# soasme/LTX-Video-GPUPoor

Measured on AMD Instinct MI355X. Metric: denoise-steps/sec + VAE-decode frames/sec, LTX-Video 768x512x97f at 1/8 GPU, higher is better.
Workload: dtype bf16

## Files before the change

### include/ltxmi.h

```cpp
#ifndef LTXMI_H
#define LTXMI_H

#include <stddef.h>
#include <stdint.h>

#ifdef __cplusplus
extern "C" {
#endif

typedef enum ltxmi_status {
    LTXMI_OK = 0,
    LTXMI_ERR_INVALID_ARG = -1,
    LTXMI_ERR_UNSUPPORTED = -2,
    LTXMI_ERR_LAUNCH = -3
} ltxmi_status;

const char* ltxmi_version(void);
const char* ltxmi_last_error(void);
const char* ltxmi_arch(void);

typedef enum ltxmi_epilogue {
    LTXMI_EPI_NONE = 0,
    LTXMI_EPI_GELU_TANH = 1,
    LTXMI_EPI_SILU = 2,
// ... 54 lines not shown
    const void* v; int64_t v_stride_b, v_stride_l;
    void*       o; int64_t o_stride_b, o_stride_l;
    const float* key_bias; int64_t bias_stride_b;
    int32_t B, H, Lq, Lk, head_dim;
    float   softmax_scale;
    const float* q_rowsumsq; int64_t q_rowsumsq_stride_b, q_rowsumsq_stride_l; int32_t q_rowsumsq_blocks;
    const void*  q_norm_weight; float q_norm_eps;
    const void*  rope_cos; const void* rope_sin; int64_t rope_stride_b, rope_stride_l;
    int32_t o_segment_len; int64_t o_stride_segment;
    const float* q_rstd; int64_t q_rstd_stride_b, q_rstd_stride_l;
    uint32_t* redo_counter; int32_t force_exact;
    float* lse; int64_t lse_stride_b, lse_stride_h;
} ltxmi_attn_args;

int ltxmi_attention_fwd_bf16(const ltxmi_attn_args* args, void* stream);
int ltxmi_attention_fuses_qnorm(int32_t B, int32_t H, int32_t Lq, int32_t Lk, int32_t head_dim, int32_t has_key_bias);
int ltxmi_attention_kernel_id(int32_t B, int32_t H, int32_t Lq, int32_t Lk, int32_t head_dim, int32_t has_key_bias,
                              int64_t k_stride_l, int64_t v_stride_l);

#define LTXMI_ATTN_MERGE_MAX 8
typedef struct ltxmi_attn_merge_args {
    int32_t n;
    const void*  o_part[LTXMI_ATTN_MERGE_MAX];   int64_t o_part_stride_b[LTXMI_ATTN_MERGE_MAX], o_part_stride_l[LTXMI_ATTN_MERGE_MAX];
    const float* lse_part[LTXMI_ATTN_MERGE_MAX]; int64_t lse_part_stride_b[LTXMI_ATTN_MERGE_MAX], lse_part_stride_h[LTXMI_ATTN_MERGE_MAX];
    void*  o;   int64_t o_stride_b, o_stride_l;
    float* lse; int64_t lse_stride_b, lse_stride_h;
    int32_t B, H, Lq, head_dim;
} ltxmi_attn_merge_args;
int ltxmi_attention_merge_bf16(const ltxmi_attn_merge_args* args, void* stream);

// ... 105 lines not shown
```

### ltx-video-gpupoor_amd/csrc/attention.h

```cpp
#pragma once
#include "common.h"

namespace ltxmi {

struct AttnParams {
    const uint16_t* q; int64_t q_sb, q_sl;
    const uint16_t* k; int64_t k_sb, k_sl;
    const uint16_t* v; int64_t v_sb, v_sl;
    uint16_t* o; int64_t o_sb, o_sl;
    const float* bias; int64_t bias_sb;
    int B, H, Lq, Lk;
    float scale_log2e;
    int q_tiles;
    const float* q_ss; int64_t q_ss_sb, q_ss_sl; int q_ss_n;
    const float* q_rstd; int64_t q_rstd_sb, q_rstd_sl;
    const uint16_t* q_w; float q_eps;
    const uint16_t* rope_cos; const uint16_t* rope_sin; int64_t rope_sb, rope_sl;
    int o_seg; int64_t o_sseg;
    uint32_t* redo_count; int force_exact;
    float* lse; int64_t lse_sb, lse_sh;

    __host__ __device__ __forceinline__ bool q_on_load() const { return q_ss != nullptr || q_rstd != nullptr; }
    __device__ __forceinline__ float q_row_rstd(int b, int row, int HD) const {
        if (q_rstd) return q_rstd[(int64_t)b * q_rstd_sb + (int64_t)row * q_rstd_sl];
// ... 146 lines not shown
}

template <typename Kern, typename... Extra>
static inline int attn_launch(Kern kern, int lds, unsigned long long* lds_done, AttnParams p, int tiles, hipStream_t stream,
                              Extra... extra) {
    if (const int rc = reserve_lds((const void*)kern, lds, lds_done, "ltxmi_attention_fwd_bf16")) return rc;
    p.q_tiles = tiles;
    const int64_t grid = (int64_t)p.B * p.H * tiles;
    hipLaunchKernelGGL(kern, dim3((unsigned)grid), dim3(256), lds, stream, p, extra...);
    return check_launch("ltxmi_attention_fwd_bf16");
}

int launch_attn_pipe(AttnParams p, hipStream_t stream);
int launch_attn_pipe128(AttnParams p, hipStream_t stream);
int launch_attn_cross(AttnParams p, hipStream_t stream);

}
```

### ltx-video-gpupoor_amd/csrc/attention.hip

```cpp
#include <type_traits>

#include "attention.h"

namespace ltxmi {

constexpr int KV_TILE = 64;
constexpr int Q_PER_WAVE = 32;
constexpr int Q_PER_WG = 128;
constexpr float LOG2E = 1.4426950408889634f;
constexpr int ATTN_QB_BIG = 2;

template <int DH>
struct AttnCfg {
    static constexpr int ROW_BYTES = DH * 2;
    static constexpr int TILE_BYTES = KV_TILE * DH * 2;
    static constexpr int CHUNKS_PER_ROW = DH / 8;
    static constexpr int LD_PER_THREAD = (KV_TILE * CHUNKS_PER_ROW) / 256;
    static constexpr int KSTEPS = DH / 16;
    static constexpr int DBLK = DH / 32;
    static constexpr int BIAS_BYTES = KV_TILE * 4;
    static constexpr int STAGE_BYTES = 2 * TILE_BYTES + BIAS_BYTES;
    static constexpr int SMEM = 2 * STAGE_BYTES;
    __device__ static __forceinline__ int k_swz(int row) {
        return DH == 64 ? ((row >> 1) & 7) : (row & 15);
// ... 329 lines not shown
    const bool span_ok = (rows * k_sl + head_dim) * 2 < (1ll << 31) && (rows * v_sl + head_dim) * 2 < (1ll << 31);
    if (head_dim == 128) {
        if (!has_bias && wg256 >= 128 && Lk >= 1024 && span_ok) return ATTN_PIPE128;
        return has_bias ? ATTN_DH128_BIAS : ATTN_DH128;
    }
    if (Lk <= ATTN_CROSS_MAX_KEYS && Lq >= 1024) return ATTN_CROSS;
    if (!has_bias && wg256 >= 192 && span_ok) return ATTN_PIPE;
    if (!has_bias && wg256 >= 512) return ATTN_DH64_QB2;
    return has_bias ? ATTN_DH64_BIAS : ATTN_DH64;
}

}

using namespace ltxmi;

extern "C" int ltxmi_attention_fwd_bf16(const ltxmi_attn_args* a, void* stream) {
    LTXMI_REQUIRE(a && a->q && a->k && a->v && a->o, LTXMI_ERR_INVALID_ARG, "ltxmi_attention_fwd_bf16: NULL argument");
    LTXMI_REQUIRE(a->B > 0 && a->H > 0 && a->Lq > 0 && a->Lk > 0, LTXMI_ERR_INVALID_ARG,
                  "ltxmi_attention_fwd_bf16: non-positive shape B=%d H=%d Lq=%d Lk=%d", a->B, a->H, a->Lq, a->Lk);
    LTXMI_REQUIRE(a->head_dim == 64 || a->head_dim == 128, LTXMI_ERR_UNSUPPORTED,
                  "ltxmi_attention_fwd_bf16: head_dim %d not in {64, 128}", a->head_dim);
    const int64_t strides[] = {a->q_stride_b, a->q_stride_l, a->k_stride_b, a->k_stride_l,
                               a->v_stride_b, a->v_stride_l, a->o_stride_b, a->o_stride_l};
    for (int64_t s : strides)
        LTXMI_REQUIRE(s % 8 == 0, LTXMI_ERR_UNSUPPORTED, "ltxmi_attention_fwd_bf16: strides must be multiples of 8 elements");
    LTXMI_REQUIRE((((uintptr_t)a->q | (uintptr_t)a->k | (uintptr_t)a->v | (uintptr_t)a->o) & 15) == 0,
                  LTXMI_ERR_UNSUPPORTED, "ltxmi_attention_fwd_bf16: q/k/v/o must be 16-byte aligned");
    LTXMI_REQUIRE((int64_t)a->B * a->H * ((a->Lq + Q_PER_WG - 1) / Q_PER_WG) < (1ll << 31), LTXMI_ERR_UNSUPPORTED,
                  "ltxmi_attention_fwd_bf16: grid too large");
    AttnParams p;
    p.q = (const uint16_t*)a->q; p.q_sb = a->q_stride_b; p.q_sl = a->q_stride_l;
    p.k = (const uint16_t*)a->k; p.k_sb = a->k_stride_b; p.k_sl = a->k_stride_l;
    p.v = (const uint16_t*)a->v; p.v_sb = a->v_stride_b; p.v_sl = a->v_stride_l;
    p.o = (uint16_t*)a->o; p.o_sb = a->o_stride_b; p.o_sl = a->o_stride_l;
    p.bias = a->key_bias; p.bias_sb = a->bias_stride_b;
    p.B = a->B; p.H = a->H; p.Lq = a->Lq; p.Lk = a->Lk;
    p.scale_log2e = a->softmax_scale * LOG2E;
    p.q_tiles = (a->Lq + Q_PER_WG - 1) / Q_PER_WG;
    p.q_ss = a->q_rowsumsq; p.q_ss_sb = a->q_rowsumsq_stride_b; p.q_ss_sl = a->q_rowsumsq_stride_l;
    p.q_ss_n = a->q_rowsumsq_blocks;
    p.q_rstd = a->q_rstd; p.q_rstd_sb = a->q_rstd_stride_b; p.q_rstd_sl = a->q_rstd_stride_l;
    p.q_w = (const uint16_t*)a->q_norm_weight; p.q_eps = a->q_norm_eps;
    p.rope_cos = (const uint16_t*)a->rope_cos; p.rope_sin = (const uint16_t*)a->rope_sin;
    p.rope_sb = a->rope_stride_b; p.rope_sl = a->rope_stride_l;
    p.o_seg = a->o_segment_len; p.o_sseg = a->o_stride_segment;
// ... 6 lines not shown
                          (a->B == 1 ? a->lse_stride_b >= 0 : a->lse_stride_b >= (int64_t)a->H * a->lse_stride_h),
                      LTXMI_ERR_INVALID_ARG,
                      "ltxmi_attention_fwd_bf16: lse must be 4-byte aligned with lse_stride_h >= Lq and lse_stride_b >= H * lse_stride_h");
    if (a->q_rowsumsq || a->q_rstd) {
        LTXMI_REQUIRE(a->q_norm_weight && (((uintptr_t)a->q_norm_weight) & 15) == 0 &&
                          (a->q_rstd ? (((uintptr_t)a->q_rstd) & 3) == 0
                                     : (a->q_rowsumsq_blocks == a->H * a->head_dim / 64 && (((uintptr_t)a->q_rowsumsq) & 3) == 0)),
                      LTXMI_ERR_INVALID_ARG, "ltxmi_attention_fwd_bf16: bad q_rowsumsq / q_rstd / q_norm_weight geometry");
        LTXMI_REQUIRE((a->rope_cos == nullptr) == (a->rope_sin == nullptr), LTXMI_ERR_INVALID_ARG,
                      "ltxmi_attention_fwd_bf16: rope_cos and rope_sin must both be given or both be NULL");
        if (a->rope_cos)
            LTXMI_REQUIRE((((uintptr_t)a->rope_cos | (uintptr_t)a->rope_sin) & 15) == 0 && a->rope_stride_l % 8 == 0 &&
                              a->rope_stride_b % 8 == 0,
                          LTXMI_ERR_INVALID_ARG, "ltxmi_attention_fwd_bf16: RoPE tables must be 16-byte aligned rows");
    }
    hipStream_t s = (hipStream_t)stream;
    switch (attn_select(a->B, a->H, a->Lq, a->Lk, a->head_dim, a->key_bias != nullptr, a->k_stride_l, a->v_stride_l)) {
        case ATTN_DH64: return launch<64, false, 1>(p, s);
        case ATTN_DH64_BIAS: return launch<64, true, 1>(p, s);
        case ATTN_DH64_QB2: return launch<64, false, ATTN_QB_BIG>(p, s);
        case ATTN_PIPE: return launch_attn_pipe(p, s);
        case ATTN_DH128: return launch<128, false, 1>(p, s);
        case ATTN_DH128_BIAS: return launch<128, true, 1>(p, s);
        case ATTN_PIPE128: return launch_attn_pipe128(p, s);
        case ATTN_CROSS: return launch_attn_cross(p, s);
    }
}

extern "C" int ltxmi_attention_kernel_id(int32_t B, int32_t H, int32_t Lq, int32_t Lk, int32_t head_dim, int32_t has_key_bias,
                                         int64_t k_stride_l, int64_t v_stride_l) {
    if (B <= 0 || H <= 0 || Lq <= 0 || Lk <= 0 || k_stride_l <= 0 || v_stride_l <= 0) return -1;
    if (head_dim != 64 && head_dim != 128) return -1;
    return attn_select(B, H, Lq, Lk, head_dim, has_key_bias != 0, k_stride_l, v_stride_l);
}

extern "C" int ltxmi_attention_fuses_qnorm(int32_t B, int32_t H, int32_t Lq, int32_t Lk, int32_t head_dim, int32_t has_key_bias) {
    return (B > 0 && H > 0 && Lq > 0 && Lk > 0 && (head_dim == 64 || head_dim == 128) && (H * head_dim) % 64 == 0) ? 1 : 0;
}
```

### ltx-video-gpupoor_amd/csrc/attention_cross.hip

```cpp
#include <type_traits>

#include "attention.h"

namespace ltxmi {

namespace cross {

#ifndef LTXMI_XATTN_STAGGER
#define LTXMI_XATTN_STAGGER 32
#endif

constexpr int DH = 64;
constexpr int KV_TILE = 64;
constexpr int MAX_TILES = 4;
constexpr int ROW_BYTES = DH * 2;
constexpr int TILE_BYTES = KV_TILE * DH * 2;
constexpr int K_OFF = 0, V_OFF = MAX_TILES * TILE_BYTES, BIAS_OFF = 2 * MAX_TILES * TILE_BYTES;
constexpr int SCR_OFF = BIAS_OFF + MAX_TILES * KV_TILE * 16;
constexpr int SCR_BYTES = 32 * 64;
constexpr int QW_OFF = SCR_OFF + 4 * SCR_BYTES;
constexpr int SMEM = QW_OFF + DH * 2;
constexpr int ROWS_PER_IT = 128;
constexpr float LOG2E = 1.4426950408889634f;

// ... 249 lines not shown
    const int nt = (p.Lk + cross::KV_TILE - 1) / cross::KV_TILE;
#define LTXMI_XATTN_LAUNCH(N)                                                                                              \
    {                                                                                                                      \
        static unsigned long long lds_done = 0;                                                                            \
        return attn_launch(cross::attn_cross_kernel<N>, cross::SMEM, &lds_done, p, groups, stream, groups, rows, n_cu);    \
    }
    switch (nt) {
        case 1: LTXMI_XATTN_LAUNCH(1)
        case 2: LTXMI_XATTN_LAUNCH(2)
        case 3: LTXMI_XATTN_LAUNCH(3)
        default: LTXMI_XATTN_LAUNCH(4)
    }
#undef LTXMI_XATTN_LAUNCH
}

}
```

### ltx-video-gpupoor_amd/ltxmi/_lib.py

```python
import ctypes
import os

import torch

_HERE = os.path.dirname(os.path.abspath(__file__))
LIB_PATH = os.environ.get("LTXMI_LIB") or os.path.join(_HERE, "libltxmi.so")

c_void_p, c_int, c_int64, c_float = ctypes.c_void_p, ctypes.c_int32, ctypes.c_int64, ctypes.c_float


class GemmArgs(ctypes.Structure):
    _fields_ = [("A", c_void_p), ("lda", c_int64), ("W", c_void_p), ("ldw", c_int64), ("bias", c_void_p),
                ("C", c_void_p), ("ldc", c_int64), ("M", c_int), ("N", c_int), ("K", c_int),
                ("epilogue", c_int), ("residual", c_void_p), ("ldr", c_int64), ("gate_table", c_void_p),
                ("gate_temb", c_void_p), ("gate_ld", c_int64), ("rows_per_group", c_int), ("algo", c_int),
                ("rowsumsq", c_void_p), ("rowsumsq_cols", c_int), ("rowsumsq_ld", c_int64),
                ("a_kblock", c_int), ("a_kblock_stride", c_int64)]


class AttnArgs(ctypes.Structure):
    _fields_ = [("q", c_void_p), ("q_stride_b", c_int64), ("q_stride_l", c_int64),
                ("k", c_void_p), ("k_stride_b", c_int64), ("k_stride_l", c_int64),
                ("v", c_void_p), ("v_stride_b", c_int64), ("v_stride_l", c_int64),
                ("o", c_void_p), ("o_stride_b", c_int64), ("o_stride_l", c_int64),
# ... 46 lines not shown
    "ltxmi_gemm_kernel_id": (c_int, [ctypes.POINTER(GemmArgs)]),
    "ltxmi_norm_modulate_bf16": (c_int, [c_void_p, c_int64, c_void_p, c_int64, c_int, c_int, c_float, c_int,
                                         c_void_p, c_void_p, c_void_p, c_void_p, c_int64, c_int, c_void_p]),
    "ltxmi_norm_modulate_f32in_bf16": (c_int, [c_void_p, c_int64, c_void_p, c_int64, c_int, c_int, c_float, c_int,
                                               c_void_p, c_void_p, c_void_p, c_void_p, c_int64, c_int, c_void_p]),
    "ltxmi_gate_residual_f32": (c_int, [c_void_p, c_int64, c_void_p, c_int64, c_int, c_int, c_void_p, c_void_p, c_int64,
                                        c_int, c_int, c_void_p, c_int64, c_void_p]),
    "ltxmi_rmsnorm_rope_bf16": (c_int, [c_void_p, c_int64, c_int, c_int, c_void_p, c_float, c_void_p, c_void_p,
                                        c_int64, c_int, c_void_p]),
    "ltxmi_rmsnorm_rope_rstd_bf16": (c_int, [c_void_p, c_int64, c_int, c_int, c_void_p, c_float, c_void_p, c_void_p,
                                             c_int64, c_int, c_void_p, c_int64, c_int, c_int, c_float, c_void_p, c_void_p]),
    "ltxmi_rowsumsq_rstd_f32": (c_int, [c_void_p, c_int64, c_int, c_int, c_int, c_float, c_void_p, c_void_p]),
    "ltxmi_qkv_norm_rope_pack_bf16": (c_int, [c_void_p, c_int64, c_int, c_int, c_int, c_int, c_void_p, c_void_p, c_float,
                                              c_void_p, c_void_p, c_int64, c_int, c_void_p, c_void_p]),
    "ltxmi_attention_fwd_bf16": (c_int, [ctypes.POINTER(AttnArgs), c_void_p]),
    "ltxmi_attention_merge_bf16": (c_int, [ctypes.POINTER(AttnMergeArgs), c_void_p]),
    "ltxmi_attention_fuses_qnorm": (c_int, [c_int, c_int, c_int, c_int, c_int, c_int]),
    "ltxmi_attention_kernel_id": (c_int, [c_int, c_int, c_int, c_int, c_int, c_int, c_int64, c_int64]),
    "ltxmi_silu_bf16": (c_int, [c_void_p, c_void_p, c_int64, c_void_p]),
    "ltxmi_timestep_embedding_bf16": (c_int, [c_void_p, c_void_p, c_int, c_int, c_void_p]),
    "ltxmi_stg_blend_bf16": (c_int, [c_void_p, c_int64, c_void_p, c_int64, c_void_p, c_int, c_int, c_int, c_void_p]),
    "ltxmi_stg_blend_grouped_bf16": (c_int, [c_void_p, c_void_p, c_int64, c_int64, c_int64, c_void_p, c_int, c_int, c_int, c_int,
                                             c_void_p]),
    "ltxmi_conv3d_ndhwc_bf16": (c_int, [ctypes.POINTER(Conv3dArgs), c_void_p]),
    "ltxmi_conv3d_fuses_post_norm": (c_int, [ctypes.POINTER(Conv3dArgs)]),
    "ltxmi_conv3d_workspace_bytes": (c_int64, [ctypes.POINTER(Conv3dArgs)]),
    "ltxmi_conv3d_route": (c_int, [ctypes.POINTER(Conv3dArgs), ctypes.POINTER(Conv3dRouteInfo)]),
    "ltxmi_pixelnorm_ada_silu_bf16": (c_int, [c_void_p, c_void_p, c_int64, c_int, c_int64, c_void_p, c_void_p,
                                              c_int, c_float, c_void_p]),
    "ltxmi_add_bf16": (c_int, [c_void_p, c_void_p, c_void_p, c_int64, c_void_p]),
# ... 53 lines not shown
```

### ltx-video-gpupoor_amd/ltxmi/attention.py

```python
from enum import Enum, auto
from typing import Optional

import torch
from torch import nn

from . import ops
from .attention_seam import pay_attention

BF16 = torch.bfloat16


FUSE_CROSS_ATTENTION_Q = True


class SkipLayerStrategy(Enum):
    AttentionSkip = auto()
    AttentionValues = auto()
    Residual = auto()
    TransformerBlock = auto()


def reshape_hidden_states(hidden_states, latent_frames):
    return hidden_states.reshape(hidden_states.shape[0], latent_frames, -1, hidden_states.shape[-1])

# ... 133 lines not shown
                              attention_mask=attention_mask, skip_layer_mask=skip_layer_mask,
                              skip_layer_strategy=skip_layer_strategy, fused_residual=fused_residual)


def _host_mask(mask):
    if mask is None:
        return None
    host = getattr(mask, "_ltxmi_host", None)
    return host if host is not None else [float(x) for x in mask.flatten().tolist()]


class AttnProcessor2_0:

    def attend(self, qkv_list, is_cross, **kw):
        return pay_attention(qkv_list, **kw)

    def __call__(self, attn: Attention, hidden_states_wrapper, freqs_cis, encoder_hidden_states=None,
                 attention_mask=None, temb=None, skip_layer_mask=None, skip_layer_strategy=None,
                 fused_residual=None, *args, **kwargs):
        hidden_states = hidden_states_wrapper[0]
        hidden_states_wrapper.clear()
        if hidden_states.dim() != 3:
            raise NotImplementedError("ltxmi.AttnProcessor2_0: only [B, N, D] inputs are on this path")
        B, N, _ = hidden_states.shape
        D = attn.inner_dim
        H = attn.heads
        dh = D // H
        x2 = hidden_states.reshape(B * N, -1)
        is_cross = encoder_hidden_states is not None
        if is_cross:
# ... 65 lines not shown
                q_fused = ((ops.rowsumsq_rstd(ss, D, attn.q_norm.eps), attn.q_norm.weight, attn.q_norm.eps), None)
            else:
                ops.rmsnorm_rope_(q2, attn.q_norm.weight, attn.q_norm.eps)
            q4 = q2.view(B, N, H, dh)
            k4 = kv.view(Bk, Lk, 2, H, dh)[:, :, 0]
            v4 = kv.view(Bk, Lk, 2, H, dh)[:, :, 1]
            v3 = kv.view(Bk, Lk, 2 * D)[:, :, D:]

        host_mask = _host_mask(skip_layer_mask) if skip_layer_mask is not None else None
        skip_attention = (host_mask is not None and skip_layer_strategy == SkipLayerStrategy.AttentionValues
                          and len(host_mask) == 1 and host_mask[0] == 0)
        if skip_attention:
            a3 = v3.contiguous()
        else:
            mask4 = None
            if attention_mask is not None:
                if attention_mask.dim() != 3 or attention_mask.shape[1] != 1:
                    raise NotImplementedError("ltxmi.AttnProcessor2_0: attention_mask must be a [B,1,Lk] bias")
                mask4 = attention_mask.reshape(B, 1, 1, Lk)
            a4 = self.attend([q4, k4, v4], is_cross, attention_mask=mask4, softmax_scale=attn.scale,
                             q_norm=q_fused[0] if q_fused else None, rope=q_fused[1] if q_fused else None)
            a3 = a4.view(B, N, D)
            if host_mask is not None and any(m != 1.0 for m in host_mask):
                m_dev = skip_layer_mask.reshape(B).to(torch.float32)
                if skip_layer_strategy == SkipLayerStrategy.AttentionValues:
                    ops.stg_blend_(a3, v3, m_dev)
                elif skip_layer_strategy == SkipLayerStrategy.AttentionSkip:
                    ops.stg_blend_(a3, hidden_states, m_dev)

        w_o, b_o = attn.to_out[0].weight, attn.to_out[0].bias
        if fused_residual is not None:
            residual, gate_table, gate_temb, rpg = fused_residual
            ops.gemm(a3.reshape(B * N, D), w_o, b_o, out=residual.reshape(B * N, -1),
                     epilogue=ops.EPI_GATE_RESIDUAL, residual=residual.reshape(B * N, -1),
                     gate_table=gate_table, gate_temb=gate_temb, rows_per_group=rpg)
            return residual
        out = ops.gemm(a3.reshape(B * N, D), w_o, b_o).view(B, N, -1)
# ... 147 lines not shown
```

### ltx-video-gpupoor_amd/ltxmi/attention_seam.py

```python
import torch

from . import ops


def _key_bias_from_mask(attention_mask, B, Lk):
    m = attention_mask
    if m.dim() != 4 or m.shape[0] != B or m.shape[-1] != Lk:
        raise ValueError(f"pay_attention: attention_mask must be [B, 1|Lq, 1|H, Lk], got {tuple(m.shape)}")
    for d in (1, 2):
        if m.shape[d] != 1 and m.stride(d) != 0:
            raise NotImplementedError(
                "pay_attention: only key biases broadcast over queries and heads are supported "
                f"(mask dim {d} has size {m.shape[d]} with stride {m.stride(d)})")
    key = (m.data_ptr(), tuple(m.shape), tuple(m.stride()), m.dtype, ops.tensor_version(m))
    hit = _BIAS_CACHE.get(key)
    if hit is None:
        if len(_BIAS_CACHE) >= 4:
            _BIAS_CACHE.clear()
        hit = _BIAS_CACHE[key] = (m[:, 0, 0, :].to(torch.float32).contiguous(), m)
    return hit[0]


_BIAS_CACHE = {}


@torch.compiler.disable()
def pay_attention(qkv_list, dropout_p=0., softmax_scale=None, causal=False, window_size=(-1, -1),
                  deterministic=False, version=None, force_attention=None, attention_mask=None,
                  cross_attn=False, q_lens=None, k_lens=None, q_norm=None, rope=None):
    q, k, v = qkv_list
    qkv_list.clear()
    if (q_norm is not None or rope is not None) and (q_lens is not None or k_lens is not None):
        raise NotImplementedError("pay_attention: q_norm / rope on load with q_lens / k_lens")
    if causal or tuple(window_size) != (-1, -1) or dropout_p != 0.:
        raise NotImplementedError("pay_attention: causal / windowed / dropout attention is not on this path")
    if force_attention not in (None, "sdpa"):
        raise NotImplementedError(f"pay_attention: backend '{force_attention}' does not exist here (single HIP backend)")
    out_dtype = q.dtype
    if v.dtype != torch.bfloat16:
        raise TypeError(f"pay_attention: bf16 only on this path, got {v.dtype}")
    q = q.to(v.dtype)
    k = k.to(v.dtype)
    b, lq, lk = q.size(0), q.size(1), k.size(1)
    final_padding = 0

    if b > 1 and k_lens is not None:
        assert attention_mask is None and q_lens is None
        k_lens = [int(x) for x in k_lens]
# ... 10 lines not shown
        k_sizes.append(cur)
        if len(chunk_sizes) > 1 or k_lens[0] != k.shape[1]:
            outs = []
            for sq, sk, sv, sz in zip(torch.split(q, chunk_sizes), torch.split(k, chunk_sizes),
                                      torch.split(v, chunk_sizes), k_sizes):
                outs.append(pay_attention([sq, sk[:, :sz], sv[:, :sz]], softmax_scale=softmax_scale))
            return torch.cat(outs, dim=0)
    elif q_lens is not None or k_lens is not None:
        assert b == 1
        szq = int(q_lens[0]) if q_lens is not None else lq
        szk = int(k_lens[0]) if k_lens is not None else lk
        final_padding = lq - szq
        q, k, v = q[:, :szq], k[:, :szk], v[:, :szk]

    bias = None if attention_mask is None else _key_bias_from_mask(attention_mask, b, k.size(1))
    x = ops.attention(q, k, v, key_bias=bias, softmax_scale=softmax_scale, q_norm=q_norm, rope=rope)
    x = x.type(out_dtype)
    if final_padding > 0:
        x = torch.cat([x, torch.empty((x.shape[0], final_padding, *x.shape[-2:]), dtype=x.dtype, device=x.device)], 1)
    return x
```

### ltx-video-gpupoor_amd/ltxmi/ops.py

```python
import ctypes
import math

import torch

from . import _lib
from ._lib import lib, check

BF16 = torch.bfloat16

EPI_NONE, EPI_GELU_TANH, EPI_SILU, EPI_GATE_RESIDUAL = 0, 1, 2, 3
NORM_RMS, NORM_LAYER = 0, 1


def _stream():
    return ctypes.c_void_p(torch.cuda.current_stream().cuda_stream)


_watch = None
_events = {}


def watch_launches(keys):
    global _watch
    _watch = set(keys) if keys else None
# ... 220 lines not shown
    check(lib.ltxmi_rowsumsq_rstd_f32(_ptr(ss), ss.stride(0), ss.shape[1], rows, norm_dim, eps, _ptr(out), _stream()),
          "ltxmi_rowsumsq_rstd_f32")
    return out


def attention_fuses_qnorm(B, H, Lq, Lk, dh, has_key_bias=False):
    return bool(lib.ltxmi_attention_fuses_qnorm(B, H, Lq, Lk, dh, int(has_key_bias)))


def attention_kernel_id(B, H, Lq, Lk, dh, has_key_bias=False, k_stride_l=None, v_stride_l=None):
    ks = 3 * H * dh if k_stride_l is None else k_stride_l
    vs = ks if v_stride_l is None else v_stride_l
    return int(lib.ltxmi_attention_kernel_id(B, H, Lq, Lk, dh, int(has_key_bias), ks, vs))


def attention(q, k, v, out=None, key_bias=None, softmax_scale=None, q_norm=None, rope=None, out_segments=None,
              redo_counter=None, force_exact=False, return_lse=False, lse=None):
    _chk_bf16(q, k, v, out)
    B, Lq, H, dh = q.shape
    Lk = k.shape[1]
    for t in (q, k, v):
        if t.stride(3) != 1 or t.stride(2) != dh:
            raise ValueError("ltxmi.attention: (heads, head_dim) must be contiguous")
    if out is None:
        if out_segments is not None:
            raise ValueError("ltxmi.attention: out_segments needs an explicit out")
        out = torch.empty((B, Lq, H, dh), dtype=BF16, device=q.device)
    if out.dim() != 4 or out.stride(3) != 1 or out.stride(2) != dh:
        raise ValueError("ltxmi.attention: out must be 4-D with (heads, head_dim) contiguous")
    a = _lib.AttnArgs()
    if out_segments is not None:
        seg_len, seg_stride = out_segments
# ... 37 lines not shown
            a.rope_stride_b = 0 if period == Lq else Lq * cos.stride(0)
    elif rope is not None:
        raise ValueError("ltxmi.attention: rope needs q_norm")
    if redo_counter is None:
        redo_counter = _redo_counter
    if redo_counter is not None:
        if redo_counter.dtype != torch.int32 or redo_counter.numel() != 1 or not redo_counter.is_cuda:
            raise ValueError("ltxmi.attention: redo_counter must be a CUDA int32 tensor of one element")
        a.redo_counter = redo_counter.data_ptr()
    a.force_exact = int(bool(force_exact))
    if return_lse or lse is not None:
        if lse is None:
            lse = torch.empty((B, H, Lq), dtype=torch.float32, device=q.device)
        _chk_lse(lse, B, H, Lq, "ltxmi.attention: lse")
        a.lse, a.lse_stride_b, a.lse_stride_h = lse.data_ptr(), lse.stride(0), lse.stride(1)
    tok = _prof_begin(("attention", B, H, Lq, Lk, dh))
    check(lib.ltxmi_attention_fwd_bf16(ctypes.byref(a), _stream()), "ltxmi_attention_fwd_bf16")
    _prof_end(tok)
    return (out, lse) if lse is not None else out


def _chk_lse(lse, B, H, Lq, what):
    if lse.dtype != torch.float32 or not lse.is_cuda or tuple(lse.shape) != (B, H, Lq) or lse.stride(2) != 1:
        raise ValueError(f"{what} must be a CUDA fp32 [B, H, Lq] = {(B, H, Lq)} tensor with contiguous tokens")


def attention_merge(outs, lses, out=None, return_lse=False, lse=None):
    n = len(outs)
    if n != len(lses) or not 2 <= n <= _lib.ATTN_MERGE_MAX:
        raise ValueError(f"ltxmi.attention_merge: {n} outputs / {len(lses)} lse tensors, need 2 .. {_lib.ATTN_MERGE_MAX} of each")
    _chk_bf16(*outs, out)
    B, Lq, H, dh = outs[0].shape
# ... 268 lines not shown


def ndhwc_to_ncdhw(x, c0, C, std=None, mean=None):
    _chk_bf16(x)
    B, T, H, W, ld = x.shape
    if not x.is_contiguous():
        raise ValueError("ltxmi.ndhwc_to_ncdhw: x must be contiguous")
    out = torch.empty((B, C, T, H, W), dtype=BF16, device=x.device)
    check(lib.ltxmi_ndhwc_to_ncdhw_bf16(_ptr(x), ld, c0, _ptr(out), B, C, T, H, W, _ptr(std), _ptr(mean), _stream()),
          "ltxmi_ndhwc_to_ncdhw_bf16")
    return out


STEP_INVARIANT_CACHING = True
STACKED_TEXT_KV = True


def set_step_invariant_caching(enabled: bool):
    global STEP_INVARIANT_CACHING
    STEP_INVARIANT_CACHING = bool(enabled)


GUIDANCE_WORKSPACE_FLOATS = 2048


def guidance_step_(noise_pred, latents, dt, guidance_scale, stg_scale, rescaling_scale, do_cfg, do_stg, do_rescale,
                   workspace, cond_mask=None, t=0.0):
    _chk_bf16(noise_pred)
    num_conds = noise_pred.shape[0]
    n = noise_pred[0].numel()
# ... 118 lines not shown
```

### ltx-video-gpupoor_amd/ltxmi/pipeline.py

```python
import copy
from dataclasses import dataclass
from typing import Any, Callable, Dict, List, Optional, Union

import torch

from . import ops
from .attention import SkipLayerStrategy
from .autoencoder import vae_decode, vae_encode
from .patchifier import SymmetricPatchifier, latent_to_pixel_coords_from_factors


@dataclass
class ConditioningItem:
    media_item: torch.Tensor
    media_frame_number: int
    conditioning_strength: float
    media_x: Optional[int] = None
    media_y: Optional[int] = None


def _refuse(rows):
    for refused, error, message in rows:
        if refused:
            raise error("ltxmi.LTXVideoPipeline: " + message)
# ... 480 lines not shown
        if not self.dead_row_elimination:
            return self.do_cfg, self.do_stg
        return (self.do_cfg and self.gs[i] > 1.0), (self.do_stg and self.stg[i] > 0.0)

    def batch(self, use_cfg, use_stg):
        key = (use_cfg, use_stg)
        if key not in self._batches:
            (e, m), (negative_e, negative_m) = self.positive, self.negative
            m = m.to(self.device)
            if use_cfg:
                e = torch.cat([negative_e, e], dim=0)
                m = torch.cat([negative_m.to(self.device), m], dim=0)
            if use_stg:
                e = torch.cat([e, self.positive[0]], dim=0)
                m = torch.cat([m, self.positive[1].to(self.device)], dim=0)
            self._batches[key] = (e.to(device=self.device, dtype=self.transformer.dtype), m, e.shape[0])
        return self._batches[key]

    def skip_mask(self, i, use_stg, nconds):
        if not use_stg or self.skip is None:
            return None
        key = (tuple(self.skip[i]), nconds)
        if key not in self._skip_masks:
            self._skip_masks[key] = self.transformer.create_skip_layer_mask(1, nconds, nconds - 1, list(self.skip[i]))
        return self._skip_masks[key]

    def stg_alias_blocks(self, i, use_stg):
        if not (self.stg_row_dedup and use_stg):
            return 0
        blocks = self.skip[i] if self.skip is not None else []
# ... 52 lines not shown
```

### ltx-video-gpupoor_amd/ltxmi/transformer3d.py

```python
import contextlib
import math
from dataclasses import dataclass
from typing import Any, Dict, List, Optional

import torch
from torch import nn

from . import ops
from .attention import BasicTransformerBlock, SkipLayerStrategy

BF16 = torch.bfloat16


@dataclass
class Transformer3DModelOutput:
    sample: torch.Tensor


class _TimestepEmbedder(nn.Module):
    def __init__(self, in_channels, dim):
        super().__init__()
        self.linear_1 = nn.Linear(in_channels, dim)
        self.linear_2 = nn.Linear(dim, dim)

# ... 134 lines not shown
        dtype = torch.float32
        dim = self.inner_dim
        theta = self.positional_embedding_theta
        frac = self.get_fractional_positions(indices_grid)
        indices = theta ** torch.linspace(math.log(1, theta), math.log(theta, theta), dim // 6,
                                          device=frac.device, dtype=dtype)
        indices = indices.to(dtype=dtype) * math.pi / 2
        freqs = (indices * (frac.unsqueeze(-1) * 2 - 1)).transpose(-1, -2).flatten(2)
        cos_freq = freqs.cos().repeat_interleave(2, dim=-1)
        sin_freq = freqs.sin().repeat_interleave(2, dim=-1)
        if dim % 6 != 0:
            cos_freq = torch.cat([torch.ones_like(cos_freq[:, :, : dim % 6]), cos_freq], dim=-1)
            sin_freq = torch.cat([torch.zeros_like(cos_freq[:, :, : dim % 6]), sin_freq], dim=-1)
        return cos_freq.to(self.dtype).contiguous(), sin_freq.to(self.dtype).contiguous()

    def _stacked_text_kv(self, ehs):
        blocks = [b for b in self.transformer_blocks if getattr(b, "attn2", None) is not None]
        if not blocks or ehs.dim() != 3 or not ehs.is_contiguous():
            return
        packs = [b.attn2.packed_kv() for b in blocks]
        if any(bk is None for _, bk in packs) or len({tuple(w.shape) for w, _ in packs}) != 1:
            return
        key = tuple((w.data_ptr(), ops.tensor_version(w), bk.data_ptr(), ops.tensor_version(bk)) for w, bk in packs)
        st = self.__dict__.get("_stacked_kv_weights")
        if st is None or st[0] != key:
            with torch.no_grad():
                st = (key, torch.cat([w for w, _ in packs], 0).contiguous(), torch.cat([bk for _, bk in packs], 0).contiguous(),
                      packs)
            self.__dict__["_stacked_kv_weights"] = st
        _, w_all, b_all, _ = st
# ... 14 lines not shown
        for block in self.transformer_blocks:
            block.prepare_shared_state()
        if on_gpu:
            main = torch.cuda.current_stream()
            key = (hidden_states.device, len(slices))
            pool = self.__dict__.setdefault("_mb_streams", {})
            streams = pool.get(key)
            if streams is None:
                streams = pool[key] = [torch.cuda.Stream(device=hidden_states.device) for _ in slices]
            for st in streams:
                st.wait_stream(main)

        def rows(t, sl):
            return t if (t is None or t.shape[0] != B) else t[sl]

        interrupted = False
        for block_idx, block in enumerate(self.transformer_blocks):
            for i, sl in enumerate(slices):
                ctx = torch.cuda.stream(streams[i]) if on_gpu else contextlib.nullcontext()
                with ctx:
                    block(hidden_states[sl], freqs_cis=tuple(rows(t, sl) for t in freqs_cis), attention_mask=attention_mask,
                          encoder_hidden_states=rows(encoder_hidden_states, sl),
                          encoder_attention_mask=rows(encoder_attention_mask, sl), timestep=temb[sl],
                          cross_attention_kwargs=cross_attention_kwargs, class_labels=class_labels,
                          skip_layer_mask=layer_mask(block_idx, sl), skip_layer_strategy=skip_layer_strategy)
            if ltxv_model is not None and ltxv_model._interrupt:
                interrupted = True
                break
        if on_gpu:
            for st in streams:
                main.wait_stream(st)
        return interrupted

    def forward(self, hidden_states: torch.Tensor, freqs_cis: list,
                encoder_hidden_states: Optional[torch.Tensor] = None, timestep: Optional[torch.Tensor] = None,
                class_labels: Optional[torch.LongTensor] = None, cross_attention_kwargs: Dict[str, Any] = None,
                attention_mask: Optional[torch.Tensor] = None, encoder_attention_mask: Optional[torch.Tensor] = None,
                skip_layer_mask: Optional[torch.Tensor] = None,
                skip_layer_strategy: Optional[SkipLayerStrategy] = None, latent_shape=None, joint_pass=True,
                ltxv_model=None, mixed=False, return_dict: bool = True, stg_alias_blocks: int = 0,
                _microbatches=None):
        if self.dtype != BF16:
            raise TypeError("ltxmi.Transformer3DModel runs in bfloat16 only: call .to(torch.bfloat16)")
        if attention_mask is not None:
            raise NotImplementedError("a self-attention mask is not on this path")
        dtype = self.dtype
        hidden_states = hidden_states.to(dtype)
        B, N, _ = hidden_states.shape
        D = self.inner_dim

        if encoder_attention_mask is not None and encoder_attention_mask.ndim == 2:
            encoder_attention_mask = ((1 - encoder_attention_mask.to(dtype)) * -10000.0).unsqueeze(1)

        hidden_states = ops.gemm(hidden_states.reshape(B * N, -1), self.patchify_proj.weight,
                                 self.patchify_proj.bias).view(B, N, D)

        timestep = timestep.to(torch.float32)
        if self.timestep_scale_multiplier:
            timestep = self.timestep_scale_multiplier * timestep
        if timestep.shape[-1] > 1:
            timestep = timestep.reshape(timestep.shape[0], -1, latent_shape[-2] * latent_shape[-1])[:, :, 0]
        temb, embedded_timestep = self.adaln_single(timestep.flatten())
        temb = temb.view(B, -1, 6 * D)
        embedded_timestep = embedded_timestep.view(B, -1, D)
        if mixed:
            hidden_states = hidden_states.float()

# ... 30 lines not shown
            return m

        first_block = 0
        if joint_pass and stg_alias_blocks and B >= 2:
            heads, dh = self.num_attention_heads, self.attention_head_dim
            if ops.attention_kernel_id(B, heads, N, N, dh) != ops.attention_kernel_id(B - 1, heads, N, N, dh):
                stg_alias_blocks = 0
        if joint_pass and stg_alias_blocks and B >= 2:
            first_block = min(int(stg_alias_blocks), len(self.transformer_blocks))
            keep = slice(0, B - 1)
            hs = hidden_states[keep]
            for block_idx in range(first_block):
                self.transformer_blocks[block_idx](
                    hs, freqs_cis=freqs_cis, attention_mask=attention_mask,
                    encoder_hidden_states=encoder_hidden_states[keep],
                    encoder_attention_mask=None if encoder_attention_mask is None else encoder_attention_mask[keep],
                    timestep=temb[keep], cross_attention_kwargs=cross_attention_kwargs, class_labels=class_labels,
                    skip_layer_mask=layer_mask(block_idx, keep), skip_layer_strategy=skip_layer_strategy)
                if ltxv_model is not None and ltxv_model._interrupt:
                    return [None]
            hidden_states[B - 1].copy_(hidden_states[B - 2])
        if joint_pass and _microbatches and len(_microbatches) > 1 and first_block == 0:
            if self._run_blocks_microbatched(hidden_states, _microbatches, freqs_cis, attention_mask, encoder_hidden_states,
                                             encoder_attention_mask, temb, cross_attention_kwargs, class_labels,
                                             layer_mask, skip_layer_strategy, ltxv_model):
                return [None]
        elif joint_pass:
            for block_idx, block in enumerate(self.transformer_blocks):
                if block_idx < first_block:
                    continue
                hidden_states = block(hidden_states, freqs_cis=freqs_cis, attention_mask=attention_mask,
                                      encoder_hidden_states=encoder_hidden_states,
                                      encoder_attention_mask=encoder_attention_mask, timestep=temb,
                                      cross_attention_kwargs=cross_attention_kwargs, class_labels=class_labels,
                                      skip_layer_mask=layer_mask(block_idx),
                                      skip_layer_strategy=skip_layer_strategy)
                if ltxv_model is not None and ltxv_model._interrupt:
                    return [None]
        else:
            for block_idx, block in enumerate(self.transformer_blocks):
                for i in range(B):
                    block(hidden_states[i:i + 1], freqs_cis=freqs_cis, attention_mask=attention_mask,
                          encoder_hidden_states=encoder_hidden_states[i:i + 1],
                          encoder_attention_mask=encoder_attention_mask[i:i + 1], timestep=temb[i:i + 1],
                          cross_attention_kwargs=cross_attention_kwargs, class_labels=class_labels,
                          skip_layer_mask=layer_mask(block_idx, slice(i, i + 1)),
                          skip_layer_strategy=skip_layer_strategy)
                    if ltxv_model is not None and ltxv_model._interrupt:
                        return [None]

        for block in self.transformer_blocks:
            if getattr(block, "attn2", None) is not None:
                block.attn2.__dict__.pop("_text_kv_ready", None)

        T1 = embedded_timestep.shape[1]
        emb2 = embedded_timestep.reshape(B * T1, D)
        if mixed:
            normed = torch.empty((B, N, D), dtype=dtype, device=hidden_states.device)
            ops.norm_modulate_f32in(hidden_states.view(B * N, D), normed.view(B * N, D), 1e-6, ops.NORM_LAYER,
# ... 10 lines not shown
```

Baseline: 16.21.

## Trim masked text keys per batch row and skip STG-perturbed self-attention rows

Host-side per-row key counts are computed once from the text attention mask, cached, and passed down to the attention entry point. There the cross-attention kernel is split into runs of batch rows with similar key-tile counts, using a cost model of launch overhead against wasted tiles, so padded keys beyond each row's last valid token are not processed. The bias kernels instead shrink Lk to the largest count. Separately, when STG uses the AttentionValues strategy with a trailing block of zero-masked rows, self-attention runs only on the kept rows and copies V into the skipped ones. The cost is extra launches, host-side planning, a one-time mask read to the host, and more complex plumbing of counts through slicing.

Measured after the change: 16.36 (median of 6 runs). About the same (+1.0%).

```diff
diff --git a/include/ltxmi.h b/include/ltxmi.h
--- a/include/ltxmi.h
+++ b/include/ltxmi.h
@@ -92,6 +92,8 @@
 } ltxmi_attn_args;
 
 int ltxmi_attention_fwd_bf16(const ltxmi_attn_args* args, void* stream);
+int ltxmi_attention_fwd_counts_bf16(const ltxmi_attn_args* args, const int32_t* host_key_counts, void* stream);
+int ltxmi_attention_launch_plan(const ltxmi_attn_args* args, const int32_t* host_key_counts, int32_t* run_rows, int32_t* run_keys);
 int ltxmi_attention_fuses_qnorm(int32_t B, int32_t H, int32_t Lq, int32_t Lk, int32_t head_dim, int32_t has_key_bias);
 int ltxmi_attention_kernel_id(int32_t B, int32_t H, int32_t Lq, int32_t Lk, int32_t head_dim, int32_t has_key_bias,
                               int64_t k_stride_l, int64_t v_stride_l);
diff --git a/ltx-video-gpupoor_amd/csrc/attention.h b/ltx-video-gpupoor_amd/csrc/attention.h
--- a/ltx-video-gpupoor_amd/csrc/attention.h
+++ b/ltx-video-gpupoor_amd/csrc/attention.h
@@ -1,4 +1,6 @@
 #pragma once
+#include <vector>
+
 #include "common.h"
 
 namespace ltxmi {
@@ -184,5 +186,25 @@
 int launch_attn_pipe(AttnParams p, hipStream_t stream);
 int launch_attn_pipe128(AttnParams p, hipStream_t stream);
 int launch_attn_cross(AttnParams p, hipStream_t stream);
-
-}
+int launch_attn_cross_counts(const AttnParams& p, const int32_t* key_counts, hipStream_t stream);
+struct AttnCrossRun {
+    int b0, rows, Lk;
+};
+std::vector<AttnCrossRun> attn_cross_plan(int B, int H, int Lq, const int32_t* key_counts);
+
+static inline AttnParams attn_batch_rows(AttnParams p, int b0, int n) {
+    p.q += (int64_t)b0 * p.q_sb;
+    p.k += (int64_t)b0 * p.k_sb;
+    p.v += (int64_t)b0 * p.v_sb;
+    p.o += (int64_t)b0 * p.o_sb;
+    if (p.bias) p.bias += (int64_t)b0 * p.bias_sb;
+    if (p.q_ss) p.q_ss += (int64_t)b0 * p.q_ss_sb;
+    if (p.q_rstd) p.q_rstd += (int64_t)b0 * p.q_rstd_sb;
+    if (p.rope_cos) p.rope_cos += (int64_t)b0 * p.rope_sb;
+    if (p.rope_sin) p.rope_sin += (int64_t)b0 * p.rope_sb;
+    if (p.lse) p.lse += (int64_t)b0 * p.lse_sb;
+    p.B = n;
+    return p;
+}
+
+}
diff --git a/ltx-video-gpupoor_amd/csrc/attention.hip b/ltx-video-gpupoor_amd/csrc/attention.hip
--- a/ltx-video-gpupoor_amd/csrc/attention.hip
+++ b/ltx-video-gpupoor_amd/csrc/attention.hip
@@ -367,7 +367,7 @@
 
 using namespace ltxmi;
 
-extern "C" int ltxmi_attention_fwd_bf16(const ltxmi_attn_args* a, void* stream) {
+static int attention_prepare(const ltxmi_attn_args* a, const int32_t* key_counts, AttnParams& p, AttnKernel& kernel) {
     LTXMI_REQUIRE(a && a->q && a->k && a->v && a->o, LTXMI_ERR_INVALID_ARG, "ltxmi_attention_fwd_bf16: NULL argument");
     LTXMI_REQUIRE(a->B > 0 && a->H > 0 && a->Lq > 0 && a->Lk > 0, LTXMI_ERR_INVALID_ARG,
                   "ltxmi_attention_fwd_bf16: non-positive shape B=%d H=%d Lq=%d Lk=%d", a->B, a->H, a->Lq, a->Lk);
@@ -381,7 +381,6 @@
                   LTXMI_ERR_UNSUPPORTED, "ltxmi_attention_fwd_bf16: q/k/v/o must be 16-byte aligned");
     LTXMI_REQUIRE((int64_t)a->B * a->H * ((a->Lq + Q_PER_WG - 1) / Q_PER_WG) < (1ll << 31), LTXMI_ERR_UNSUPPORTED,
                   "ltxmi_attention_fwd_bf16: grid too large");
-    AttnParams p;
     p.q = (const uint16_t*)a->q; p.q_sb = a->q_stride_b; p.q_sl = a->q_stride_l;
     p.k = (const uint16_t*)a->k; p.k_sb = a->k_stride_b; p.k_sl = a->k_stride_l;
     p.v = (const uint16_t*)a->v; p.v_sb = a->v_stride_b; p.v_sl = a->v_stride_l;
@@ -418,8 +417,25 @@
                               a->rope_stride_b % 8 == 0,
                           LTXMI_ERR_INVALID_ARG, "ltxmi_attention_fwd_bf16: RoPE tables must be 16-byte aligned rows");
     }
+    int max_count = 0;
+    if (key_counts)
+        for (int b = 0; b < a->B; ++b) {
+            const int32_t n = key_counts[b];
+            LTXMI_REQUIRE(n >= 1 && n <= a->Lk, LTXMI_ERR_INVALID_ARG,
+                          "ltxmi_attention_fwd_bf16: key_counts[%d] = %d outside 1 .. Lk = %d", b, n, a->Lk);
+            max_count = n > max_count ? n : max_count;
+        }
+    kernel = attn_select(a->B, a->H, a->Lq, a->Lk, a->head_dim, a->key_bias != nullptr, a->k_stride_l, a->v_stride_l);
+    if (key_counts && (kernel == ATTN_DH64_BIAS || kernel == ATTN_DH128_BIAS)) p.Lk = max_count;
+    return LTXMI_OK;
+}
+
+static int attention_fwd(const ltxmi_attn_args* a, const int32_t* key_counts, void* stream) {
+    AttnParams p;
+    AttnKernel kernel;
+    if (const int rc = attention_prepare(a, key_counts, p, kernel)) return rc;
     hipStream_t s = (hipStream_t)stream;
-    switch (attn_select(a->B, a->H, a->Lq, a->Lk, a->head_dim, a->key_bias != nullptr, a->k_stride_l, a->v_stride_l)) {
+    switch (kernel) {
         case ATTN_DH64: return launch<64, false, 1>(p, s);
         case ATTN_DH64_BIAS: return launch<64, true, 1>(p, s);
         case ATTN_DH64_QB2: return launch<64, false, ATTN_QB_BIG>(p, s);
@@ -427,8 +443,33 @@
         case ATTN_DH128: return launch<128, false, 1>(p, s);
         case ATTN_DH128_BIAS: return launch<128, true, 1>(p, s);
         case ATTN_PIPE128: return launch_attn_pipe128(p, s);
-        case ATTN_CROSS: return launch_attn_cross(p, s);
-    }
+        case ATTN_CROSS: return key_counts ? launch_attn_cross_counts(p, key_counts, s) : launch_attn_cross(p, s);
+    }
+}
+
+extern "C" int ltxmi_attention_fwd_bf16(const ltxmi_attn_args* a, void* stream) { return attention_fwd(a, nullptr, stream); }
+
+extern "C" int ltxmi_attention_fwd_counts_bf16(const ltxmi_attn_args* a, const int32_t* host_key_counts, void* stream) {
+    return attention_fwd(a, host_key_counts, stream);
+}
+
+extern "C" int ltxmi_attention_launch_plan(const ltxmi_attn_args* a, const int32_t* host_key_counts, int32_t* run_rows,
+                                           int32_t* run_keys) {
+    LTXMI_REQUIRE(run_rows && run_keys, LTXMI_ERR_INVALID_ARG, "ltxmi_attention_launch_plan: NULL argument");
+    AttnParams p;
+    AttnKernel kernel;
+    if (const int rc = attention_prepare(a, host_key_counts, p, kernel)) return rc;
+    if (kernel != ATTN_CROSS || !host_key_counts) {
+        run_rows[0] = p.B;
+        run_keys[0] = p.Lk;
+        return 1;
+    }
+    const std::vector<AttnCrossRun> runs = attn_cross_plan(p.B, p.H, p.Lq, host_key_counts);
+    for (size_t i = 0; i < runs.size(); ++i) {
+        run_rows[i] = runs[i].rows;
+        run_keys[i] = runs[i].Lk;
+    }
+    return (int)runs.size();
 }
 
 extern "C" int ltxmi_attention_kernel_id(int32_t B, int32_t H, int32_t Lq, int32_t Lk, int32_t head_dim, int32_t has_key_bias,
diff --git a/ltx-video-gpupoor_amd/csrc/attention_cross.hip b/ltx-video-gpupoor_amd/csrc/attention_cross.hip
--- a/ltx-video-gpupoor_amd/csrc/attention_cross.hip
+++ b/ltx-video-gpupoor_amd/csrc/attention_cross.hip
@@ -287,4 +287,42 @@
 #undef LTXMI_XATTN_LAUNCH
 }
 
-}
+std::vector<AttnCrossRun> attn_cross_plan(int B, int H, int Lq, const int32_t* key_counts) {
+    auto tiles = [](int count) { return (count + cross::KV_TILE - 1) / cross::KV_TILE; };
+    std::vector<AttnCrossRun> runs;
+    for (int b = 0; b < B; ++b) {
+        const int nt = tiles(key_counts[b]);
+        if (!runs.empty() && tiles(runs.back().Lk) == nt) {
+            runs.back().rows += 1;
+            runs.back().Lk = key_counts[b] > runs.back().Lk ? key_counts[b] : runs.back().Lk;
+        } else {
+            runs.push_back(AttnCrossRun{b, 1, key_counts[b]});
+        }
+    }
+    const double launch_us = 13.0, row_tile_us = 3.44 * ((double)H * Lq) / (32.0 * 4992.0);
+    for (;;) {
+        int best = -1;
+        double best_gain = 0.0;
+        for (size_t i = 0; i + 1 < runs.size(); ++i) {
+            const int na = tiles(runs[i].Lk), nb = tiles(runs[i + 1].Lk), nm = na > nb ? na : nb;
+            const double gain = launch_us - row_tile_us * (runs[i].rows * (nm - na) + runs[i + 1].rows * (nm - nb));
+            if (gain > best_gain) best = (int)i, best_gain = gain;
+        }
+        if (best < 0) break;
+        runs[best].rows += runs[best + 1].rows;
+        runs[best].Lk = runs[best + 1].Lk > runs[best].Lk ? runs[best + 1].Lk : runs[best].Lk;
+        runs.erase(runs.begin() + best + 1);
+    }
+    return runs;
+}
+
+int launch_attn_cross_counts(const AttnParams& p, const int32_t* key_counts, hipStream_t stream) {
+    for (const AttnCrossRun& r : attn_cross_plan(p.B, p.H, p.Lq, key_counts)) {
+        AttnParams run = attn_batch_rows(p, r.b0, r.rows);
+        run.Lk = r.Lk;
+        if (const int rc = launch_attn_cross(run, stream)) return rc;
+    }
+    return LTXMI_OK;
+}
+
+}
diff --git a/ltx-video-gpupoor_amd/ltxmi/_lib.py b/ltx-video-gpupoor_amd/ltxmi/_lib.py
--- a/ltx-video-gpupoor_amd/ltxmi/_lib.py
+++ b/ltx-video-gpupoor_amd/ltxmi/_lib.py
@@ -84,6 +84,9 @@
     "ltxmi_qkv_norm_rope_pack_bf16": (c_int, [c_void_p, c_int64, c_int, c_int, c_int, c_int, c_void_p, c_void_p, c_float,
                                               c_void_p, c_void_p, c_int64, c_int, c_void_p, c_void_p]),
     "ltxmi_attention_fwd_bf16": (c_int, [ctypes.POINTER(AttnArgs), c_void_p]),
+    "ltxmi_attention_fwd_counts_bf16": (c_int, [ctypes.POINTER(AttnArgs), ctypes.POINTER(c_int), c_void_p]),
+    "ltxmi_attention_launch_plan": (c_int, [ctypes.POINTER(AttnArgs), ctypes.POINTER(c_int), ctypes.POINTER(c_int),
+                                            ctypes.POINTER(c_int)]),
     "ltxmi_attention_merge_bf16": (c_int, [ctypes.POINTER(AttnMergeArgs), c_void_p]),
     "ltxmi_attention_fuses_qnorm": (c_int, [c_int, c_int, c_int, c_int, c_int, c_int]),
     "ltxmi_attention_kernel_id": (c_int, [c_int, c_int, c_int, c_int, c_int, c_int, c_int64, c_int64]),
diff --git a/ltx-video-gpupoor_amd/ltxmi/attention.py b/ltx-video-gpupoor_amd/ltxmi/attention.py
--- a/ltx-video-gpupoor_amd/ltxmi/attention.py
+++ b/ltx-video-gpupoor_amd/ltxmi/attention.py
@@ -171,6 +171,19 @@
 
     def attend(self, qkv_list, is_cross, **kw):
         return pay_attention(qkv_list, **kw)
+
+    def _stg_kept_rows(self, B, H, N, dh, host_mask, skip_layer_strategy):
+        if (not ops.STG_SKIP_ROWS or host_mask is None or skip_layer_strategy != SkipLayerStrategy.AttentionValues
+                or len(host_mask) != B or type(self).attend is not AttnProcessor2_0.attend):
+            return B
+        kept = 0
+        while kept < B and host_mask[kept] == 1.0:
+            kept += 1
+        if kept == 0 or kept == B or any(m != 0.0 for m in host_mask[kept:]):
+            return B
+        if ops.attention_kernel_id(B, H, N, N, dh) != ops.attention_kernel_id(kept, H, N, N, dh):
+            return B
+        return kept
 
     def __call__(self, attn: Attention, hidden_states_wrapper, freqs_cis, encoder_hidden_states=None,
                  attention_mask=None, temb=None, skip_layer_mask=None, skip_layer_strategy=None,
@@ -266,13 +279,30 @@
             a3 = v3.contiguous()
         else:
             mask4 = None
+            extra = {}
             if attention_mask is not None:
                 if attention_mask.dim() != 3 or attention_mask.shape[1] != 1:
                     raise NotImplementedError("ltxmi.AttnProcessor2_0: attention_mask must be a [B,1,Lk] bias")
                 mask4 = attention_mask.reshape(B, 1, 1, Lk)
-            a4 = self.attend([q4, k4, v4], is_cross, attention_mask=mask4, softmax_scale=attn.scale,
-                             q_norm=q_fused[0] if q_fused else None, rope=q_fused[1] if q_fused else None)
-            a3 = a4.view(B, N, D)
+                counts = getattr(attention_mask, "_ltxmi_key_counts", None)
+                if counts is not None and len(counts) == B:
+                    extra["key_counts"] = counts
+            q_norm, rope = (q_fused[0], q_fused[1]) if q_fused else (None, None)
+            kept = self._stg_kept_rows(B, H, N, dh, host_mask, skip_layer_strategy) if not is_cross and mask4 is None else B
+            if kept < B:
+                if q_norm is not None:
+                    q_norm = (q_norm[0][:kept * N],) + tuple(q_norm[1:])
+                if rope is not None and rope[2] == B * N:
+                    rope = (rope[0][:kept * N], rope[1][:kept * N], kept * N)
+                a3 = torch.empty((B, N, D), dtype=q4.dtype, device=q4.device)
+                self.attend([q4[:kept], k4[:kept], v4[:kept]], is_cross, attention_mask=None, softmax_scale=attn.scale,
+                            q_norm=q_norm, rope=rope, out=a3[:kept].view(kept, N, H, dh))
+                a3[kept:].copy_(v3[kept:])
+                host_mask = None
+            else:
+                a4 = self.attend([q4, k4, v4], is_cross, attention_mask=mask4, softmax_scale=attn.scale,
+                                 q_norm=q_norm, rope=rope, **extra)
+                a3 = a4.view(B, N, D)
             if host_mask is not None and any(m != 1.0 for m in host_mask):
                 m_dev = skip_layer_mask.reshape(B).to(torch.float32)
                 if skip_layer_strategy == SkipLayerStrategy.AttentionValues:
diff --git a/ltx-video-gpupoor_amd/ltxmi/attention_seam.py b/ltx-video-gpupoor_amd/ltxmi/attention_seam.py
--- a/ltx-video-gpupoor_amd/ltxmi/attention_seam.py
+++ b/ltx-video-gpupoor_amd/ltxmi/attention_seam.py
@@ -27,11 +27,14 @@
 @torch.compiler.disable()
 def pay_attention(qkv_list, dropout_p=0., softmax_scale=None, causal=False, window_size=(-1, -1),
                   deterministic=False, version=None, force_attention=None, attention_mask=None,
-                  cross_attn=False, q_lens=None, k_lens=None, q_norm=None, rope=None):
+                  cross_attn=False, q_lens=None, k_lens=None, q_norm=None, rope=None, key_counts=None,
+                  out=None):
     q, k, v = qkv_list
     qkv_list.clear()
     if (q_norm is not None or rope is not None) and (q_lens is not None or k_lens is not None):
         raise NotImplementedError("pay_attention: q_norm / rope on load with q_lens / k_lens")
+    if out is not None and (q_lens is not None or k_lens is not None):
+        raise NotImplementedError("pay_attention: out with q_lens / k_lens")
     if causal or tuple(window_size) != (-1, -1) or dropout_p != 0.:
         raise NotImplementedError("pay_attention: causal / windowed / dropout attention is not on this path")
     if force_attention not in (None, "sdpa"):
@@ -72,7 +75,12 @@
         q, k, v = q[:, :szq], k[:, :szk], v[:, :szk]
 
     bias = None if attention_mask is None else _key_bias_from_mask(attention_mask, b, k.size(1))
-    x = ops.attention(q, k, v, key_bias=bias, softmax_scale=softmax_scale, q_norm=q_norm, rope=rope)
+    extra = {}
+    if out is not None:
+        extra["out"] = out
+    if key_counts is not None and bias is not None and bias.is_cuda:
+        extra["key_counts"] = key_counts
+    x = ops.attention(q, k, v, key_bias=bias, softmax_scale=softmax_scale, q_norm=q_norm, rope=rope, **extra)
     x = x.type(out_dtype)
     if final_padding > 0:
         x = torch.cat([x, torch.empty((x.shape[0], final_padding, *x.shape[-2:]), dtype=x.dtype, device=x.device)], 1)
diff --git a/ltx-video-gpupoor_amd/ltxmi/ops.py b/ltx-video-gpupoor_amd/ltxmi/ops.py
--- a/ltx-video-gpupoor_amd/ltxmi/ops.py
+++ b/ltx-video-gpupoor_amd/ltxmi/ops.py
@@ -258,8 +258,25 @@
     return int(lib.ltxmi_attention_kernel_id(B, H, Lq, Lk, dh, int(has_key_bias), ks, vs))
 
 
+def attention_launch_plan(B, H, Lq, Lk, dh, key_counts=None, has_key_bias=True):
+    a = _lib.AttnArgs()
+    a.q = a.k = a.v = a.o = 1 << 30
+    a.key_bias = (1 << 30) if has_key_bias else None
+    a.bias_stride_b = Lk
+    a.B, a.H, a.Lq, a.Lk, a.head_dim, a.softmax_scale = B, H, Lq, Lk, dh, 1.0 / math.sqrt(dh)
+    a.q_stride_l = a.k_stride_l = a.v_stride_l = a.o_stride_l = H * dh
+    a.q_stride_b = a.o_stride_b = Lq * H * dh
+    a.k_stride_b = a.v_stride_b = Lk * H * dh
+    counts = None if key_counts is None else (ctypes.c_int32 * B)(*[int(n) for n in key_counts])
+    rows, keys = (ctypes.c_int32 * B)(), (ctypes.c_int32 * B)()
+    n = lib.ltxmi_attention_launch_plan(ctypes.byref(a), counts, rows, keys)
+    if n < 0:
+        check(n, "ltxmi_attention_launch_plan")
+    return [(rows[i], keys[i]) for i in range(n)]
+
+
 def attention(q, k, v, out=None, key_bias=None, softmax_scale=None, q_norm=None, rope=None, out_segments=None,
-              redo_counter=None, force_exact=False, return_lse=False, lse=None):
+              redo_counter=None, force_exact=False, return_lse=False, lse=None, key_counts=None):
     _chk_bf16(q, k, v, out)
     B, Lq, H, dh = q.shape
     Lk = k.shape[1]
@@ -327,8 +344,16 @@
             lse = torch.empty((B, H, Lq), dtype=torch.float32, device=q.device)
         _chk_lse(lse, B, H, Lq, "ltxmi.attention: lse")
         a.lse, a.lse_stride_b, a.lse_stride_h = lse.data_ptr(), lse.stride(0), lse.stride(1)
+    counts = None
+    if key_counts is not None and KEY_COUNTS:
+        if key_bias is None or len(key_counts) != B:
+            raise ValueError("ltxmi.attention: key_counts is a host list of B entries and comes with the key_bias that removes those keys")
+        counts = (ctypes.c_int32 * B)(*[int(n) for n in key_counts])
     tok = _prof_begin(("attention", B, H, Lq, Lk, dh))
-    check(lib.ltxmi_attention_fwd_bf16(ctypes.byref(a), _stream()), "ltxmi_attention_fwd_bf16")
+    if counts is None:
+        check(lib.ltxmi_attention_fwd_bf16(ctypes.byref(a), _stream()), "ltxmi_attention_fwd_bf16")
+    else:
+        check(lib.ltxmi_attention_fwd_counts_bf16(ctypes.byref(a), counts, _stream()), "ltxmi_attention_fwd_counts_bf16")
     _prof_end(tok)
     return (out, lse) if lse is not None else out
 
@@ -627,6 +652,19 @@
 
 STEP_INVARIANT_CACHING = True
 STACKED_TEXT_KV = True
+KEY_COUNTS = True
+STG_SKIP_ROWS = True
+
+
+def key_counts_from_mask(mask):
+    if mask.dim() != 2:
+        raise ValueError(f"ltxmi.key_counts_from_mask: expected a [B, Lk] mask, got {tuple(mask.shape)}")
+    Lk = mask.shape[1]
+    counts = []
+    for row in (mask != 0).cpu().tolist():
+        last = max((i for i, on in enumerate(row) if on), default=-1)
+        counts.append(last + 1 if last >= 0 else Lk)
+    return counts
 
 
 def set_step_invariant_caching(enabled: bool):
diff --git a/ltx-video-gpupoor_amd/ltxmi/pipeline.py b/ltx-video-gpupoor_amd/ltxmi/pipeline.py
--- a/ltx-video-gpupoor_amd/ltxmi/pipeline.py
+++ b/ltx-video-gpupoor_amd/ltxmi/pipeline.py
@@ -518,6 +518,10 @@
             if use_stg:
                 e = torch.cat([e, self.positive[0]], dim=0)
                 m = torch.cat([m, self.positive[1].to(self.device)], dim=0)
+            if m.dim() == 2:
+                if m is self.positive[1]:
+                    m = m.clone()
+                m._ltxmi_key_counts = ops.key_counts_from_mask(m)
             self._batches[key] = (e.to(device=self.device, dtype=self.transformer.dtype), m, e.shape[0])
         return self._batches[key]
 
diff --git a/ltx-video-gpupoor_amd/ltxmi/transformer3d.py b/ltx-video-gpupoor_amd/ltxmi/transformer3d.py
--- a/ltx-video-gpupoor_amd/ltxmi/transformer3d.py
+++ b/ltx-video-gpupoor_amd/ltxmi/transformer3d.py
@@ -172,6 +172,21 @@
             sin_freq = torch.cat([torch.zeros_like(cos_freq[:, :, : dim % 6]), sin_freq], dim=-1)
         return cos_freq.to(self.dtype).contiguous(), sin_freq.to(self.dtype).contiguous()
 
+    def _mask_key_counts(self, mask):
+        counts = getattr(mask, "_ltxmi_key_counts", None)
+        if counts is not None and len(counts) == mask.shape[0]:
+            return list(counts)
+        if not ops.KEY_COUNTS:
+            return None
+        key = (mask.data_ptr(), tuple(mask.shape), tuple(mask.stride()), mask.dtype, ops.tensor_version(mask))
+        cache = self.__dict__.setdefault("_key_count_cache", {})
+        hit = cache.get(key)
+        if hit is None:
+            if len(cache) >= 4:
+                cache.clear()
+            hit = cache[key] = (ops.key_counts_from_mask(mask), mask)
+        return hit[0]
+
     def _stacked_text_kv(self, ehs):
         blocks = [b for b in self.transformer_blocks if getattr(b, "attn2", None) is not None]
         if not blocks or ehs.dim() != 3 or not ehs.is_contiguous():
@@ -216,6 +231,13 @@
         def rows(t, sl):
             return t if (t is None or t.shape[0] != B) else t[sl]
 
+        def mask_rows(sl):
+            m = rows(encoder_attention_mask, sl)
+            counts = getattr(encoder_attention_mask, "_ltxmi_key_counts", None)
+            if counts is not None and m is not encoder_attention_mask:
+                m._ltxmi_key_counts = counts[sl]
+            return m
+
         interrupted = False
         for block_idx, block in enumerate(self.transformer_blocks):
             for i, sl in enumerate(slices):
@@ -223,7 +245,7 @@
                 with ctx:
                     block(hidden_states[sl], freqs_cis=tuple(rows(t, sl) for t in freqs_cis), attention_mask=attention_mask,
                           encoder_hidden_states=rows(encoder_hidden_states, sl),
-                          encoder_attention_mask=rows(encoder_attention_mask, sl), timestep=temb[sl],
+                          encoder_attention_mask=mask_rows(sl), timestep=temb[sl],
                           cross_attention_kwargs=cross_attention_kwargs, class_labels=class_labels,
                           skip_layer_mask=layer_mask(block_idx, sl), skip_layer_strategy=skip_layer_strategy)
             if ltxv_model is not None and ltxv_model._interrupt:
@@ -251,8 +273,22 @@
         B, N, _ = hidden_states.shape
         D = self.inner_dim
 
+        key_counts = None
         if encoder_attention_mask is not None and encoder_attention_mask.ndim == 2:
+            key_counts = self._mask_key_counts(encoder_attention_mask)
             encoder_attention_mask = ((1 - encoder_attention_mask.to(dtype)) * -10000.0).unsqueeze(1)
+
+        def bias_rows(sl=None):
+            m = encoder_attention_mask
+            if m is None:
+                return None
+            if m.shape[0] != B:
+                return m
+            if sl is not None:
+                m = m[sl]
+            if key_counts is not None:
+                m._ltxmi_key_counts = key_counts if sl is None else key_counts[sl]
+            return m
 
         hidden_states = ops.gemm(hidden_states.reshape(B * N, -1), self.patchify_proj.weight,
                                  self.patchify_proj.bias).view(B, N, D)
@@ -313,7 +349,7 @@
                 self.transformer_blocks[block_idx](
                     hs, freqs_cis=freqs_cis, attention_mask=attention_mask,
                     encoder_hidden_states=encoder_hidden_states[keep],
-                    encoder_attention_mask=None if encoder_attention_mask is None else encoder_attention_mask[keep],
+                    encoder_attention_mask=bias_rows(keep),
                     timestep=temb[keep], cross_attention_kwargs=cross_attention_kwargs, class_labels=class_labels,
                     skip_layer_mask=layer_mask(block_idx, keep), skip_layer_strategy=skip_layer_strategy)
                 if ltxv_model is not None and ltxv_model._interrupt:
@@ -321,7 +357,7 @@
             hidden_states[B - 1].copy_(hidden_states[B - 2])
         if joint_pass and _microbatches and len(_microbatches) > 1 and first_block == 0:
             if self._run_blocks_microbatched(hidden_states, _microbatches, freqs_cis, attention_mask, encoder_hidden_states,
-                                             encoder_attention_mask, temb, cross_attention_kwargs, class_labels,
+                                             bias_rows(), temb, cross_attention_kwargs, class_labels,
                                              layer_mask, skip_layer_strategy, ltxv_model):
                 return [None]
         elif joint_pass:
@@ -330,7 +366,7 @@
                     continue
                 hidden_states = block(hidden_states, freqs_cis=freqs_cis, attention_mask=attention_mask,
                                       encoder_hidden_states=encoder_hidden_states,
-                                      encoder_attention_mask=encoder_attention_mask, timestep=temb,
+                                      encoder_attention_mask=bias_rows(), timestep=temb,
                                       cross_attention_kwargs=cross_attention_kwargs, class_labels=class_labels,
                                       skip_layer_mask=layer_mask(block_idx),
                                       skip_layer_strategy=skip_layer_strategy)
@@ -341,7 +377,7 @@
                 for i in range(B):
                     block(hidden_states[i:i + 1], freqs_cis=freqs_cis, attention_mask=attention_mask,
                           encoder_hidden_states=encoder_hidden_states[i:i + 1],
-                          encoder_attention_mask=encoder_attention_mask[i:i + 1], timestep=temb[i:i + 1],
+                          encoder_attention_mask=bias_rows(slice(i, i + 1)), timestep=temb[i:i + 1],
                           cross_attention_kwargs=cross_attention_kwargs, class_labels=class_labels,
                           skip_layer_mask=layer_mask(block_idx, slice(i, i + 1)),
                           skip_layer_strategy=skip_layer_strategy)
```
